# Keep-Passion/ImageStitch

Hardware: AMD Instinct MI355X
Metric: image-pairs/sec (2048x2048 grayscale, SURF+BF) (higher is better)
Workload: dtype f32

## Files before the change

imagestitch_amd/csrc/surf_kernels.hip:

```cpp
#include "common.h"
#include "detmath.h"
#include <math.h>
#include <float.h>
#include <string.h>
#include <stdlib.h>
#include <algorithm>
#include <vector>

#define GAS __attribute__((address_space(1)))
typedef GAS const uint8_t *g_cu8;
typedef GAS const int32_t *g_ci32;
typedef GAS float *g_f32;
typedef GAS const float *g_cf32;
typedef GAS int32_t *g_i32;
__device__ __forceinline__ int cv_round_f(float v) { return (int)rintf(v); }
__device__ __forceinline__ uint8_t round_u8_pos(float v) { return (uint8_t)__float_as_uint(v + 12582912.f); }
__device__ __forceinline__ int cv_round_d(double v) { return (int)rint(v); }
__device__ __forceinline__ int cv_floor_d(double v) { return (int)floor(v); }
__device__ __forceinline__ int cv_ceil_d(double v) { return (int)ceil(v); }

__device__ __forceinline__ int wave_incl_scan(int v)
{
    const int lane = threadIdx.x & 63;
#pragma unroll
// ... 863 lines not shown
#pragma unroll
                for (int off = 32; off >= 1; off >>= 1) {
                    const float om = __shfl_xor(bm, off, 64); const int oi = __shfl_xor(bi, off, 64);
                    if (om > bm || (om == bm && oi < bi)) { bm = om; bi = oi; }
                }
                if (lane == 0) {
                    float bestx = 0, besty = 0;
                    if (bm > 0.f) { bestx = sx_s[q][bi]; besty = sy_s[q][bi]; }
                    R.kps[k].angle = fast_atan2_deg(-besty, bestx);
                }
            }
        }
    }
}

#ifdef VFSMS_DESC_TIMING
__device__ unsigned long long g_desc_cycles[8];
#define DT_MARK(ph) do { if (threadIdx.x == 0) { unsigned long long _n = clock64(); atomicAdd(&g_desc_cycles[ph], _n - _t0); _t0 = _n; } } while (0)
#define DT_START unsigned long long _t0 = clock64()
extern "C" int vfsms_debug_desc_cycles(unsigned long long *out) { return hipMemcpyFromSymbol(out, HIP_SYMBOL(g_desc_cycles), sizeof(unsigned long long) * 8) == hipSuccess ? 0 : -3; }
__device__ unsigned long long g_desc_trips[4];
#define DT_TRIP(n) do {} while (0)
__device__ unsigned long long g_desc_unit_cycles[4];
#define DT_UNIT_BEGIN unsigned long long _u0 = clock64()
#define DT_UNIT_END(n) do { _uacc[n] += clock64() - _u0; _ucnt[n]++; } while (0)
extern "C" int vfsms_debug_desc_unit_cycles(unsigned long long *out) { return hipMemcpyFromSymbol(out, HIP_SYMBOL(g_desc_unit_cycles), sizeof(unsigned long long) * 4) == hipSuccess ? 0 : -3; }
extern "C" int vfsms_debug_desc_trips(unsigned long long *out) { return hipMemcpyFromSymbol(out, HIP_SYMBOL(g_desc_trips), sizeof(unsigned long long) * 4) == hipSuccess ? 0 : -3; }
#else
#define DT_MARK(ph) do {} while (0)
#define DT_START do {} while (0)
#define DT_TRIP(n) do {} while (0)
#define DT_UNIT_BEGIN do {} while (0)
#define DT_UNIT_END(n) do {} while (0)
#endif
#ifndef VFSMS_EXP
#define VFSMS_EXP 0
#endif
#ifndef DESC_WBUF
#define DESC_WBUF 15360
#endif
__device__ __forceinline__ void origin_chain(float *row, float s, const float d, const int n)
{
    int i = 0;
    for (; i + 4 <= n; i += 4) {
        const float a = s, b = a + d, c = b + d, e = c + d;
        s = e + d;
        row[i] = a; row[i + 1] = b; row[i + 2] = c; row[i + 3] = e;
    }
    for (; i < n; i++, s += d) row[i] = s;
}

struct WinGeom {
    int win; float sin_dir, cos_dir;
    int h, w, stride; g_cu8 img;
    g_cu8 pair;
    int upright, usx, usy;
};

__device__ __forceinline__ int win_sample_xy(const WinGeom &G, double px, double py)
{
    const int ncols1 = G.w - 1, nrows1 = G.h - 1;
    const int ix = (int)px, iy = (int)py;
    if (px >= 0.0 && py >= 0.0 && ix < ncols1 && iy < nrows1) {
        const float a = (float)__builtin_amdgcn_fract(px), b = (float)__builtin_amdgcn_fract(py);
        g_cu8 p = G.img + (size_t)iy * G.stride + ix;
        const float v = p[0] * (1.f - a) * (1.f - b) + p[1] * a * (1.f - b) + p[G.stride] * (1.f - a) * b + p[G.stride + 1] * a * b;
        return (int)(uint8_t)cv_round_f(v);
    }
    const int x = min(max(cv_round_d(px), 0), ncols1);
    const int y = min(max(cv_round_d(py), 0), nrows1);
    return (int)G.img[(size_t)y * G.stride + x];
}
__device__ __forceinline__ int win_sample_upright(const WinGeom &G, int i, int j)
{
    const int x = min(max(G.usx + i, 0), G.w - 1);
    const int y = min(max(G.usy - j, 0), G.h - 1);
    return (int)G.img[(size_t)y * G.stride + x];
}

typedef float float2v __attribute__((ext_vector_type(2)));
__device__ __forceinline__ float bilinear_pk(uint32_t top, float a, float b)
{
    const float na = 1.f - a, nb = 1.f - b;
    const float2v w = {na, a};
    const float2v r0 = {(float)(top & 0xff), (float)((top >> 16) & 0xff)};
    const float2v r1 = {(float)((top >> 8) & 0xff), (float)(top >> 24)};
    float2v p = r0 * w, q = r1 * w;
    const float2v nb2 = {nb, nb}, b2 = {b, b};
    p = p * nb2; q = q * b2;
    return ((p.x + p.y) + q.x) + q.y;
}
#ifndef STAGE_ILP
#define STAGE_ILP 4
#endif
#define UNIT_W (8 * STAGE_ILP)
#ifndef BORDER_ILP
#define BORDER_ILP 2
#endif
#ifndef STAGE_FRAC_FIRST
#define STAGE_FRAC_FIRST 1
#endif
template <int N>
__device__ __forceinline__ void stage_round(g_cu8 ubase, const uint32_t pw, const double c, const double sn, const double sxc, const double syc,
                                            const int jlane, uint8_t *wrow)
{
    uint32_t top[N];
    const double jd = (double)jlane;
    const double px0 = __builtin_fma(jd, c, sxc), py0 = __builtin_fma(jd, -sn, syc);
#if STAGE_FRAC_FIRST
    float fa[N], fb[N];
#pragma unroll
    for (int u = 0; u < N; u++) {
        const double px = u ? px0 + (double)(8 * u) * c : px0, py = u ? py0 - (double)(8 * u) * sn : py0;
        const uint32_t off = ((uint32_t)__umul24((uint32_t)(int)py, pw) + (uint32_t)(int)px) << 1;
        fa[u] = (float)__builtin_amdgcn_fract(px); fb[u] = (float)__builtin_amdgcn_fract(py);
        top[u] = *(GAS const uint32_t *)(ubase + off);
    }
#pragma unroll
    for (int u = 0; u < N; u++) wrow[8 * u] = round_u8_pos(bilinear_pk(top[u], fa[u], fb[u]));
#else
    double px[N], py[N];
    px[0] = px0; py[0] = py0;
#pragma unroll
    for (int u = 1; u < N; u++) { px[u] = px[0] + (double)(8 * u) * c; py[u] = py[0] - (double)(8 * u) * sn; }
#pragma unroll
    for (int u = 0; u < N; u++) {
        const uint32_t off = ((uint32_t)__umul24((uint32_t)(int)py[u], pw) + (uint32_t)(int)px[u]) << 1;
        top[u] = *(GAS const uint32_t *)(ubase + off);
    }
#pragma unroll
    for (int u = 0; u < N; u++) {
        const float a = (float)__builtin_amdgcn_fract(px[u]), b = (float)__builtin_amdgcn_fract(py[u]);
        wrow[8 * u] = round_u8_pos(bilinear_pk(top[u], a, b));
    }
#endif
}

template <int NW>
__device__ __forceinline__ void stage_rows(const WinGeom &G, const float *sx_row, const float *sy_row,
                                           int r0, int nrows, uint8_t *dst, uint8_t *strip_in)
{
    const int win = __builtin_amdgcn_readfirstlane(G.win);
    r0 = __builtin_amdgcn_readfirstlane(r0); nrows = __builtin_amdgcn_readfirstlane(nrows);
    const int lane = threadIdx.x & 63, wv = NW == 1 ? 0 : __builtin_amdgcn_readfirstlane((int)(threadIdx.x >> 6));
    const int li = lane >> 3, lj = lane & 7;
    const int strips = (nrows + 7) >> 3;
    const double c = (double)G.cos_dir, sn = (double)G.sin_dir;
    const int ncols1 = __builtin_amdgcn_readfirstlane(G.w) - 1, nrows1 = __builtin_amdgcn_readfirstlane(G.h) - 1;
    const uint64_t bp = (uint64_t)G.pair;
    g_cu8 ubase = (g_cu8)(((uint64_t)(uint32_t)__builtin_amdgcn_readfirstlane((uint32_t)(bp >> 32)) << 32) |
                          (uint64_t)(uint32_t)__builtin_amdgcn_readfirstlane((uint32_t)bp));
    const uint32_t pw = (uint32_t)(ncols1 + 1);
    const int gfull = win >> 3, tailc = win & 7;
    int nb = NW == 1 ? 1 : (gfull + 7) >> 3;
#if VFSMS_EXP & 16
    nb = (gfull + 3) >> 2;
#endif
    const int gbase = gfull / nb, grem = gfull - gbase * nb;
    const int total = strips * nb;
    if (!G.upright) {
        const int tid = NW == 1 ? lane : (int)threadIdx.x;
        if (tid < strips) {
            const int ia = min(r0 + tid * 8, VFSMS_MAX_WIN - 1), ib = min(min(r0 + tid * 8 + 7, r0 + nrows - 1), VFSMS_MAX_WIN - 1);
            const double xa = (double)sx_row[ia], xb = (double)sx_row[ib], ya = (double)sy_row[ia], yb = (double)sy_row[ib];
            const double jb = (double)(win - 1);
            const double jxb = jb * c, jyb = -(jb * sn);
            const double xmin = fmin(xa, xb) + fmin(0.0, jxb), xmax = fmax(xa, xb) + fmax(0.0, jxb);
            const double ymin = fmin(ya, yb) + fmin(0.0, jyb), ymax = fmax(ya, yb) + fmax(0.0, jyb);
            strip_in[tid] = xmin >= 0.0 && ymin >= 0.0 && xmax < (double)(ncols1 - 2) && ymax < (double)nrows1;
        }
        if (NW == 1) { __builtin_amdgcn_fence(__ATOMIC_ACQ_REL, "wavefront"); __builtin_amdgcn_wave_barrier(); }
        else __syncthreads();
    }
    int ty = 0, cbi = wv;
    while (cbi >= nb) { cbi -= nb; ty++; }
#ifdef VFSMS_DESC_TIMING
    unsigned long long _s0 = clock64(), _uacc[2] = {0, 0}, _ucnt[2] = {0, 0};
#endif
    const int last_row = r0 + nrows - 1;
    const int liw = li * win;
    const int last_off = (nrows - 1) * win;
    float nsx = 0.f, nsy = 0.f; int nflag = 0;
    if (wv < total) {
        const int ic0 = min(r0 + ty * 8 + li, last_row);
        nsx = sx_row[ic0]; nsy = sy_row[ic0]; nflag = strip_in[ty];
    }
    for (int unit = wv; unit < total; unit += NW) {
        DT_UNIT_BEGIN;
        const int g0 = cbi * gbase + min(cbi, grem), gn = gbase + (cbi < grem ? 1 : 0);
        const bool last_run = cbi == nb - 1;
        const int cb0 = g0 * 8;
        const int cb1 = last_run ? win : cb0 + gn * 8;
        const double sxc = (double)nsx, syc = (double)nsy;
        const int flag_cur = nflag;
        const int ty_cur = ty;
        uint8_t *drc = dst + min(ty * 8 * win + liw, last_off);
        cbi += NW;
        while (cbi >= nb) { cbi -= nb; ty++; }
        if (unit + NW < total) {
            const int icn = min(r0 + ty * 8 + li, last_row);
            nsx = sx_row[icn]; nsy = sy_row[icn]; nflag = strip_in[ty];
        }
        if (G.upright) {
            for (int j = cb0 + lj; j < cb1; j += 8) drc[j] = (uint8_t)win_sample_upright(G, min(r0 + ty_cur * 8 + li, last_row), j);
            continue;
        }
        bool unit_in = __builtin_amdgcn_readfirstlane(flag_cur) != 0;
        if (!unit_in) {
            const int ia = min(r0 + ty_cur * 8, VFSMS_MAX_WIN - 1), ib = min(min(r0 + ty_cur * 8 + 7, last_row), VFSMS_MAX_WIN - 1);
            const double xa = (double)sx_row[ia], xb = (double)sx_row[ib], ya = (double)sy_row[ia], yb = (double)sy_row[ib];
            const double ja = (double)cb0, jb = (double)(cb1 - 1);
            const double jxa = ja * c, jxb = jb * c, jya = -(ja * sn), jyb = -(jb * sn);
            const double xmin = fmin(xa, xb) + fmin(jxa, jxb), xmax = fmax(xa, xb) + fmax(jxa, jxb);
            const double ymin = fmin(ya, yb) + fmin(jya, jyb), ymax = fmax(ya, yb) + fmax(jya, jyb);
            unit_in = xmin >= 0.0 && ymin >= 0.0 && xmax < (double)(ncols1 - 2) && ymax < (double)nrows1;
        }
        if (unit_in) {
            DT_TRIP(0);
            uint8_t *wrow = drc + cb0 + lj;
            int jl = cb0 + lj, left = gn;
            while (left >= 4) { stage_round<4>(ubase, pw, c, sn, sxc, syc, jl, wrow); jl += 32; wrow += 32; left -= 4; }
            if (left == 3) stage_round<3>(ubase, pw, c, sn, sxc, syc, jl, wrow);
            else if (left == 2) stage_round<2>(ubase, pw, c, sn, sxc, syc, jl, wrow);
            else if (left == 1) stage_round<1>(ubase, pw, c, sn, sxc, syc, jl, wrow);
            if (last_run && tailc) {
                const int jc = min(gfull * 8 + lj, win - 1);
                stage_round<1>(ubase, pw, c, sn, sxc, syc, jc, drc + jc);
            }
            DT_UNIT_END(0);
            continue;
        }
        DT_TRIP(2);
        for (int jb = cb0; jb < cb1; jb += 8 * BORDER_ILP) {
            double px[BORDER_ILP], py[BORDER_ILP];
            int jc[BORDER_ILP];
            uint32_t top[BORDER_ILP];
            bool inside[BORDER_ILP];
#pragma unroll
            for (int u = 0; u < BORDER_ILP; u++) {
                jc[u] = min(jb + u * 8 + lj, cb1 - 1);
                px[u] = sxc + (double)jc[u] * c;
                py[u] = syc - (double)jc[u] * sn;
                const int ix = (int)px[u], iy = (int)py[u];
                inside[u] = px[u] >= 0.0 && py[u] >= 0.0 && ix < ncols1 && iy < nrows1;
                const int rx = min(max(cv_round_d(px[u]), 0), ncols1), ry = min(max(cv_round_d(py[u]), 0), nrows1);
                const int cx = inside[u] ? ix : rx, cy = inside[u] ? iy : ry;
                top[u] = *(GAS const uint32_t *)(ubase + (((uint32_t)__umul24((uint32_t)cy, pw) + (uint32_t)cx) << 1));
            }
#pragma unroll
            for (int u = 0; u < BORDER_ILP; u++) {
                const float a = (float)__builtin_amdgcn_fract(px[u]), b = (float)__builtin_amdgcn_fract(py[u]);
                const float v = (float)(top[u] & 0xff) * (1.f - a) * (1.f - b) + (float)((top[u] >> 16) & 0xff) * a * (1.f - b) +
                                (float)((top[u] >> 8) & 0xff) * (1.f - a) * b + (float)(top[u] >> 24) * a * b;
                drc[jc[u]] = inside[u] ? (uint8_t)cv_round_f(v) : (uint8_t)(top[u] & 0xff);
            }
        }
        DT_UNIT_END(1);
    }
#ifdef VFSMS_DESC_TIMING
    if ((threadIdx.x & 63) == 0) {
        atomicAdd(&g_desc_unit_cycles[2], clock64() - _s0);
        atomicAdd(&g_desc_unit_cycles[0], _uacc[0]); atomicAdd(&g_desc_unit_cycles[1], _uacc[1]);
        atomicAdd(&g_desc_trips[0], _ucnt[0]); atomicAdd(&g_desc_trips[2], _ucnt[1]);
    }
#endif
}

__device__ __forceinline__ uint8_t sat_u8(float v)
{
    int iv = cv_round_f(v);
    return (uint8_t)(iv < 0 ? 0 : iv > 255 ? 255 : iv);
}

struct AreaRec { int j0, n; float a0, af, al; int mode, r1, r2; };
#define AREA_RECS 22

__device__ __forceinline__ float area_row_tab(const uint8_t *S, const AreaRec &c, const int nmin, const int nmax)
{
    const uint8_t *p = S + c.j0;
    float buf = (float)p[0] * c.a0;
    int t = 1;
    for (; t < nmin - 1; t++) buf += (float)p[t] * c.af;
    for (; t < nmax; t++) buf += (float)p[t] * (t < c.n - 1 ? c.af : (t == c.n - 1 ? c.al : 0.f));
    return buf;
}
#define AREA_TAIL 4
__device__ __forceinline__ void area_tail_weights(const AreaRec &c, const int nmin, float (&w)[AREA_TAIL])
{
    const int t0 = max(nmin - 1, 1);
#pragma unroll
    for (int i = 0; i < AREA_TAIL; i++) w[i] = t0 + i < c.n - 1 ? c.af : (t0 + i == c.n - 1 ? c.al : 0.f);
}
__device__ __forceinline__ float area_row_tab_w(const uint8_t *S, const AreaRec &c, const int nmin, const int nmax, const float (&w)[AREA_TAIL])
{
    const uint8_t *p = S + c.j0;
    float buf = (float)p[0] * c.a0;
    int t = 1;
    for (; t < nmin - 1; t++) buf += (float)p[t] * c.af;
#pragma unroll
    for (int i = 0; i < AREA_TAIL; i++)
        if (t + i < nmax) buf += (float)p[t + i] * w[i];
    return buf;
}
__device__ __forceinline__ uint8_t area_col_tab(const float *rb, const AreaRec &c, const int mode, const float inv_area)
{
    float sum = c.a0 * rb[0];
    for (int t = 1; t < c.n; t++) sum += (t < c.n - 1 ? c.af : c.al) * rb[t * 21];
    if (mode == 2) return (uint8_t)(((int)sum + 2) >> 2);
    if (mode == 1) return sat_u8(sum * inv_area);
    return sat_u8(sum);
}

__device__ void describe_one(const RoiDev &R, const SurfTables *T, const AreaRec *area_tab, const DescRec &rec, int extended, int upright, const int band)
{
    DT_START;
    const int k = rec.k;
    __shared__ float sx_row[VFSMS_MAX_WIN], sy_row[VFSMS_MAX_WIN];
    __shared__ uint8_t PATCH[21][21 + 3];
    __shared__ AreaRec REC[AREA_RECS];
    __shared__ uint8_t WINBUF[DESC_WBUF];
    __shared__ float rowsum[40 * 21];
    __shared__ uint8_t STRIP_IN[VFSMS_MAX_WIN / 8 + 8];
    WinGeom G;
    G.win = max(21, min(rec.win, VFSMS_MAX_WIN));
    G.h = R.h; G.w = R.w; G.stride = R.stride; G.img = (g_cu8)R.img; G.pair = (g_cu8)R.pair;
    G.upright = upright; G.usx = 0; G.usy = 0; G.sin_dir = rec.sin_dir; G.cos_dir = rec.cos_dir;
    const int win = G.win;
    const int dsz = 21;
    if (threadIdx.x < AREA_RECS * 8) ((int *)REC)[threadIdx.x] = ((const int *)(area_tab + (size_t)win * AREA_RECS))[threadIdx.x];
    __syncthreads();
    const int nmin = __builtin_amdgcn_readfirstlane(REC[21].j0), nmax = __builtin_amdgcn_readfirstlane(REC[21].n);
    const int mode = __builtin_amdgcn_readfirstlane(REC[21].mode);
    const float inv_area = REC[21].a0;
    if (!upright) {
        if (threadIdx.x == 0 || threadIdx.x == 64) {
            const float sin_dir = rec.sin_dir, cos_dir = rec.cos_dir;
            const float win_offset = -(float)(win - 1) / 2;
            const int need = band >= 0 ? min(win, REC[band].j0 + REC[band].n) : win;
            if (threadIdx.x == 0) origin_chain(sx_row, rec.x + win_offset * cos_dir + win_offset * sin_dir, sin_dir, need);
            else origin_chain(sy_row, rec.y - win_offset * sin_dir + win_offset * cos_dir, cos_dir, need);
        }
    } else {
        const float win_offset = -(float)(win - 1) / 2;
        G.usx = cv_round_f(rec.x + win_offset);
        G.usy = cv_round_f(rec.y - win_offset);
    }
    __syncthreads();
    DT_MARK(0);

    const bool tail_ok = nmax - max(nmin - 1, 1) <= AREA_TAIL;
    auto reduce_rows = [&](const int st_lo, int dyA, const int dy_stop) {
        while (dyA < dy_stop) {
            const int lo = REC[dyA].j0;
            int dyB = dyA + 1;
            while (dyB < dy_stop && REC[dyB].j0 + REC[dyB].n - lo <= 40) dyB++;
            const int nr = REC[dyB - 1].j0 + REC[dyB - 1].n - lo;
            for (int e = threadIdx.x; e < nr * 21; e += 256) {
                const int r = (int)(((uint32_t)e * 3121u) >> 16), dx = e - 21 * r;
                if (tail_ok) {
                    const AreaRec cx = REC[dx];
                    float w[AREA_TAIL];
                    area_tail_weights(cx, nmin, w);
                    rowsum[e] = area_row_tab_w(WINBUF + (lo - st_lo + r) * win, cx, nmin, nmax, w);
                } else
                    rowsum[e] = area_row_tab(WINBUF + (lo - st_lo + r) * win, REC[dx], nmin, nmax);
            }
            __syncthreads();
            for (int o = threadIdx.x; o < (dyB - dyA) * 21; o += 256) {
                const int dyl = (int)(((uint32_t)o * 3121u) >> 16), dx = o - 21 * dyl;
                const AreaRec ry = REC[dyA + dyl];
                PATCH[dyA + dyl][dx] = area_col_tab(rowsum + (ry.j0 - lo) * 21 + dx, ry, mode, inv_area);
            }
            __syncthreads();
            dyA = dyB;
        }
    };
    if (win * win <= DESC_WBUF) {
        stage_rows<4>(G, sx_row, sy_row, 0, win, WINBUF, STRIP_IN);
        __syncthreads();
        DT_MARK(1);
        reduce_rows(0, 0, dsz);
        DT_MARK(2);
    } else {
        const int dy_end = band >= 0 ? band + 1 : dsz;
        const int crows = max(DESC_WBUF / win, 1);
        for (int dy = band >= 0 ? band : 0; dy < dy_end;) {
            const int rlo = REC[dy].j0, nrows = REC[dy].n;
            if (nrows <= crows) {
                int d_stop = dy + 1;
                while (d_stop < dy_end && REC[d_stop].j0 + REC[d_stop].n - rlo <= crows) d_stop++;
                const int end = REC[d_stop - 1].j0 + REC[d_stop - 1].n - 1;
                stage_rows<4>(G, sx_row, sy_row, rlo, end - rlo + 1, WINBUF, STRIP_IN);
                __syncthreads();
                DT_MARK(3);
                reduce_rows(rlo, dy, d_stop);
                DT_MARK(4);
                dy = d_stop;
            } else {
                for (int c0 = 0; c0 < nrows; c0 += crows) {
                    const int cn = min(crows, nrows - c0);
                    stage_rows<4>(G, sx_row, sy_row, rlo + c0, cn, WINBUF, STRIP_IN);
                    __syncthreads();
                    DT_MARK(3);
                    for (int e = threadIdx.x; e < cn * 21; e += 256) {
                        const int r = (int)(((uint32_t)e * 3121u) >> 16), dx = e - 21 * r;
                        rowsum[c0 * 21 + e] = area_row_tab(WINBUF + r * win, REC[dx], nmin, nmax);
                    }
                    __syncthreads();
                }
                if (threadIdx.x < dsz) PATCH[dy][threadIdx.x] = area_col_tab(rowsum + threadIdx.x, REC[dy], mode, inv_area);
                __syncthreads();
                DT_MARK(4);
                dy++;
            }
        }
    }
    __syncthreads();
    if (band >= 0) {
        if (threadIdx.x < 21) R.patch[(size_t)k * VFSMS_PATCH_ROW + band * 21 + threadIdx.x] = PATCH[band][threadIdx.x];
    } else {
        for (int o = threadIdx.x; o < 441; o += 256) R.patch[(size_t)k * VFSMS_PATCH_ROW + o] = PATCH[o / 21][o % 21];
    }
    DT_MARK(5);
}

#define DESC_NCLS 4

__device__ __forceinline__ int desc_class(float size)
{
    const float s = size * 1.2f / 9.0f;
    const int win = min((int)((20 + 1) * s), VFSMS_MAX_WIN);
    return win > 256 ? 0 : win > 128 ? 1 : win > 64 ? 2 : 3;
}

__global__ __launch_bounds__(1024) void k_desc_order(const RoiDev *rois)
{
    const RoiDev &R = rois[blockIdx.x];
    const int n = min(R.counters[0], R.cap);
    __shared__ int cnt[DESC_NCLS], base[DESC_NCLS], cur[DESC_NCLS];
    if (threadIdx.x < DESC_NCLS) { cnt[threadIdx.x] = 0; cur[threadIdx.x] = 0; }
    __syncthreads();
    const int lane = threadIdx.x & 63;
    for (int k0 = 0; k0 < n; k0 += 1024) {
        const int k = k0 + threadIdx.x;
        const float size = k < n ? R.kps[k].size : -1.f;
        const int cls = size > 0 ? desc_class(size) : -1;
#pragma unroll
        for (int c = 0; c < DESC_NCLS; c++) {
            const unsigned long long m = __ballot(cls == c);
            if (m && lane == __ffsll((long long)m) - 1) atomicAdd(&cnt[c], __popcll(m));
        }
    }
    __syncthreads();
    if (threadIdx.x == 0) {
        int acc = 0;
        for (int c = 0; c < DESC_NCLS; c++) { base[c] = acc; acc += cnt[c]; R.counters[12 + c] = cnt[c]; }
    }
    __syncthreads();
    for (int k0 = 0; k0 < n; k0 += 1024) {
        const int k = k0 + threadIdx.x;
        const float size = k < n ? R.kps[k].size : -1.f;
        const int cls = size > 0 ? desc_class(size) : -1;
#pragma unroll
        for (int c = 0; c < DESC_NCLS; c++) {
            const unsigned long long m = __ballot(cls == c);
            if (!m) continue;
            const int leader = __ffsll((long long)m) - 1;
            int start = 0;
            if (lane == leader) start = atomicAdd(&cur[c], __popcll(m));
            start = __shfl(start, leader, 64);
            if (cls == c) R.order[base[c] + start + __popcll(m & ((1ull << lane) - 1))] = k;
        }
    }
}

#define DESC_HEADS DESC_PLAN_HEADS
#define DESC_HEAD_STRIDE 64

__global__ __launch_bounds__(256) void k_desc_plan(const RoiDev *rois, int nrois, DescPlan *plan, int big_grid)
{
    __shared__ int c[VFSMS_MAX_ROIS][4];
    for (int e = threadIdx.x; e < nrois * 4; e += 256) c[e >> 2][e & 3] = rois[e >> 2].counters[12 + (e & 3)];
    __syncthreads();
    if (threadIdx.x == 0) {
        int acc = 0, total = 0;
        for (int q = 0; q < DESC_HEADS; q++) {
            plan->big_start[q] = acc;
            for (int r = q; r < nrois; r += DESC_HEADS) { plan->seg_base[r][0] = acc; acc += c[r][0]; }
            plan->big_n0[q] = acc - plan->big_start[q];
            for (int r = q; r < nrois; r += DESC_HEADS) {
                plan->seg_base[r][1] = acc; acc += c[r][1];
                plan->seg_base[r][2] = acc; acc += c[r][2];
            }
            plan->big_tickets[q] = acc - plan->big_start[q];
        }
        total = acc;
        const int split = total < big_grid * 48 ? 21 : 1;
        plan->split = split;
        for (int q = 0; q < DESC_HEADS; q++) plan->big_tickets[q] += (split - 1) * plan->big_n0[q];
        acc = 0;
        for (int q = 0; q < DESC_HEADS; q++) {
            plan->small_start[q] = acc;
            for (int r = q; r < nrois; r += DESC_HEADS) { plan->seg_base[r][3] = acc; acc += c[r][3]; }
            plan->small_tickets[q] = acc - plan->small_start[q];
        }
    }
}

__global__ __launch_bounds__(256) void k_desc_recs(const RoiDev *rois, const DescPlan *plan, DescRec *big, DescRec *small, int upright)
{
    const int roi = blockIdx.y;
    const RoiDev &R = rois[roi];
    const int p = blockIdx.x * 256 + threadIdx.x;
    const int c0 = R.counters[12], c1 = R.counters[13], c2 = R.counters[14], c3 = R.counters[15];
    if (p >= c0 + c1 + c2 + c3) return;
    const int cls = p < c0 ? 0 : p < c0 + c1 ? 1 : p < c0 + c1 + c2 ? 2 : 3;
    const int idx = p - (cls > 0 ? c0 : 0) - (cls > 1 ? c1 : 0) - (cls > 2 ? c2 : 0);
    const int k = R.order[p];
    const vfsms_keypoint kp = R.kps[k];
    DescRec rec;
    rec.roi = roi; rec.k = k; rec.pad = 0; rec.x = kp.x; rec.y = kp.y;
    rec.win = (int)((20 + 1) * (kp.size * 1.2f / 9.0f));
    rec.sin_dir = 0.f; rec.cos_dir = 0.f;
    if (!upright) {
        const float dir = kp.angle * (float)(3.1415926535897932384626433832795 / 180);
        double sd, cd;
        det_sincos((double)dir, &sd, &cd);
        rec.sin_dir = -(float)sd;
        rec.cos_dir = (float)cd;
    }
    (cls < 3 ? big : small)[plan->seg_base[roi][cls] + idx] = rec;
}

__global__ __launch_bounds__(ORI_KP * 128, 8) void k_orientation(const RoiDev *rois, const SurfTables *T, int upright)
{
    const RoiDev &R = rois[blockIdx.y];
    const int n = min(R.counters[0], R.cap);
    const int k0 = blockIdx.x * ORI_KP;
    if (k0 >= n) return;
    orientation_block(R, T, k0, n, upright);
}

#define DESC_SMALL_WIN 64
struct SmallLds { uint8_t win[DESC_SMALL_WIN * DESC_SMALL_WIN + 64]; float sx[DESC_SMALL_WIN + 8], sy[DESC_SMALL_WIN + 8]; AreaRec rec[AREA_RECS]; int rec_win; uint8_t strip_in[DESC_SMALL_WIN / 8 + 8]; };

__device__ __forceinline__ void wave_sync_lds()
{
    __builtin_amdgcn_fence(__ATOMIC_ACQ_REL, "wavefront");
    __builtin_amdgcn_wave_barrier();
}

__device__ void describe_small(const RoiDev &R, const AreaRec *area_tab, const DescRec &rec, int upright, SmallLds &L)
{
    const int lane = threadIdx.x & 63;
    const int k = rec.k;
    WinGeom G;
    G.win = min(rec.win, DESC_SMALL_WIN);
    G.h = R.h; G.w = R.w; G.stride = R.stride; G.img = (g_cu8)R.img; G.pair = (g_cu8)R.pair;
    G.upright = upright; G.usx = 0; G.usy = 0; G.sin_dir = rec.sin_dir; G.cos_dir = rec.cos_dir;
    const int win = G.win;
    const int dsz = 21;
    if (L.rec_win != win) {
        wave_sync_lds();
        const int *src = (const int *)(area_tab + (size_t)max(win, dsz) * AREA_RECS);
        for (int e = lane; e < AREA_RECS * 8; e += 64) ((int *)L.rec)[e] = src[e];
        if (lane == 0) L.rec_win = win;
    }
    if (!upright) {
        const float sin_dir = rec.sin_dir, cos_dir = rec.cos_dir;
        if (lane < 2) {
            const float win_offset = -(float)(win - 1) / 2;
            const float sx0 = rec.x + win_offset * cos_dir + win_offset * sin_dir, sy0 = rec.y - win_offset * sin_dir + win_offset * cos_dir;
            origin_chain(lane == 0 ? L.sx : L.sy, lane == 0 ? sx0 : sy0, lane == 0 ? sin_dir : cos_dir, win);
        }
    } else {
        const float win_offset = -(float)(win - 1) / 2;
        G.usx = cv_round_f(rec.x + win_offset);
        G.usy = cv_round_f(rec.y - win_offset);
    }
    wave_sync_lds();
    stage_rows<1>(G, L.sx, L.sy, 0, win, L.win, L.strip_in);
    wave_sync_lds();
    const int nmin = __builtin_amdgcn_readfirstlane(L.rec[21].j0), nmax = __builtin_amdgcn_readfirstlane(L.rec[21].n);
    const int mode = __builtin_amdgcn_readfirstlane(L.rec[21].mode);
    const float inv_area = L.rec[21].a0;
    const bool tail_ok = nmax - max(nmin - 1, 1) <= AREA_TAIL;
    uint8_t *prow = R.patch + (size_t)k * VFSMS_PATCH_ROW;
    for (int o = lane; o < dsz * dsz; o += 64) {
        const int dy = (int)(((uint32_t)o * 3121u) >> 16), dx = o - dsz * dy;
        const AreaRec ry = L.rec[dy], rx = L.rec[dx];
        const uint8_t *S = L.win + ry.j0 * win;
        float sum;
        if (tail_ok) {
            float w[AREA_TAIL];
            area_tail_weights(rx, nmin, w);
            sum = ry.a0 * area_row_tab_w(S, rx, nmin, nmax, w);
            for (int ty = 1; ty < nmax; ty++) {
                const float beta = ty < ry.n - 1 ? ry.af : (ty == ry.n - 1 ? ry.al : 0.f);
                sum += beta * area_row_tab_w(S + ty * win, rx, nmin, nmax, w);
            }
        } else {
            sum = ry.a0 * area_row_tab(S, rx, nmin, nmax);
            for (int ty = 1; ty < nmax; ty++) {
                const float beta = ty < ry.n - 1 ? ry.af : (ty == ry.n - 1 ? ry.al : 0.f);
                sum += beta * area_row_tab(S + ty * win, rx, nmin, nmax);
            }
        }
        uint8_t outv;
        if (mode == 2) outv = (uint8_t)(((int)sum + 2) >> 2);
        else if (mode == 1) outv = sat_u8(sum * inv_area);
        else outv = sat_u8(sum);
        prow[o] = outv;
    }
    wave_sync_lds();
}

#ifndef DESC_SMALL_WGS
#define DESC_SMALL_WGS 7
#endif
__device__ __forceinline__ DescRec load_rec_uniform(const DescRec *p)
{
    const int *q = (const int *)p;
    DescRec r;
    r.roi = __builtin_amdgcn_readfirstlane(q[0]); r.k = __builtin_amdgcn_readfirstlane(q[1]);
    r.win = __builtin_amdgcn_readfirstlane(q[2]); r.pad = 0;
    r.sin_dir = __int_as_float(__builtin_amdgcn_readfirstlane(q[4])); r.cos_dir = __int_as_float(__builtin_amdgcn_readfirstlane(q[5]));
    r.x = __int_as_float(__builtin_amdgcn_readfirstlane(q[6])); r.y = __int_as_float(__builtin_amdgcn_readfirstlane(q[7]));
    return r;
}
__global__ __launch_bounds__(256, DESC_SMALL_WGS) void k_describe_small(const RoiDev *rois, const DescPlan *plan, const DescRec *recs, int *counter,
                                                                 const AreaRec *area_tab, int upright)
{
    __shared__ SmallLds L[4];
    if (threadIdx.x < 4) L[threadIdx.x].rec_win = -1;
    __syncthreads();
    const int lane = threadIdx.x & 63, wave = __builtin_amdgcn_readfirstlane((int)(threadIdx.x >> 6));
    int head = 0;
    for (;;) {
        int slot = -1;
        if (lane == 0)
            while (head < DESC_HEADS) {
                const int q = (blockIdx.x + head) & (DESC_HEADS - 1);
                const int n = plan->small_tickets[q];
                const int t = n > 0 ? atomicAdd(counter + q * DESC_HEAD_STRIDE, 1) : 0;
                if (t < n) { slot = plan->small_start[q] + t; break; }
                head++;
            }
        slot = __builtin_amdgcn_readfirstlane(slot);
        head = __builtin_amdgcn_readfirstlane(head);
        if (slot < 0) break;
        const DescRec rec = load_rec_uniform(recs + slot);
        describe_small(rois[rec.roi], area_tab, rec, upright, L[wave]);
    }
}

__global__ __launch_bounds__(256) void k_pair_rows(const RoiDev *rois)
{
    const RoiDev &R = rois[blockIdx.z];
    const int y = blockIdx.y, x = (blockIdx.x * 256 + threadIdx.x) * 4;
    if (y >= R.h || x >= R.w) return;
    g_cu8 r0 = (g_cu8)R.img + (size_t)y * R.stride + x, r1 = (g_cu8)R.img + (size_t)min(y + 1, R.h - 1) * R.stride + x;
    GAS uint16_t *dst = (GAS uint16_t *)R.pair + (size_t)y * R.w + x;
    if (x + 4 <= R.w) {
        const uint32_t a = *(GAS const u32u *)r0, b = *(GAS const u32u *)r1;
#pragma unroll
        for (int k = 0; k < 4; k++) dst[k] = (uint16_t)(((a >> (8 * k)) & 0xff) | (((b >> (8 * k)) & 0xff) << 8));
    } else {
        for (int k = 0; x + k < R.w; k++) dst[k] = (uint16_t)(r0[k] | (r1[k] << 8));
    }
}

#ifndef DESC_WGS
#define DESC_WGS 6
#endif
__global__ __launch_bounds__(256, DESC_WGS) void k_describe(const RoiDev *rois, const DescPlan *plan, const DescRec *recs, int *counter, const SurfTables *T,
                                                  const AreaRec *area_tab, int extended, int upright)
{
    __shared__ int s_slot, s_band;
    int head = 0;
#ifdef VFSMS_DESC_TIMING
    unsigned long long tq = clock64();
#endif
    for (;;) {
        __syncthreads();
        if (threadIdx.x == 0) {
            int slot = -1, band = -1;
            const int split = plan->split;
            while (head < DESC_HEADS) {
                const int q = (blockIdx.x + head) & (DESC_HEADS - 1);
                const int n = plan->big_tickets[q];
                const int t = n > 0 ? atomicAdd(counter + q * DESC_HEAD_STRIDE, 1) : 0;
                if (t < n) {
                    const int n0 = plan->big_n0[q];
                    if (t < n0 * split) { slot = plan->big_start[q] + t / split; band = split > 1 ? t % split : -1; }
                    else slot = plan->big_start[q] + n0 + (t - n0 * split);
                    break;
                }
                head++;
            }
            s_slot = slot; s_band = band;
        }
        __syncthreads();
        const int slot = __builtin_amdgcn_readfirstlane(s_slot), band = __builtin_amdgcn_readfirstlane(s_band);
        if (slot < 0) break;
#ifdef VFSMS_DESC_TIMING
        if (threadIdx.x == 0) atomicAdd(&g_desc_cycles[6], clock64() - tq);
#endif
        const DescRec rec = load_rec_uniform(recs + slot);
        describe_one(rois[rec.roi], T, area_tab, rec, extended, upright, band);
#ifdef VFSMS_DESC_TIMING
        tq = clock64();
#endif
    }
}

__global__ __launch_bounds__(1024) void k_keep_scan(const RoiDev *rois)
{
// ... 318 lines not shown
```

Measured before the change: 2304.

## Stream large descriptor windows in uniform row chunks with running column accumulators

Replaces the per-output-row staging of oversized descriptor windows with a single pass over the needed row range, in chunks sized to leave room for a 441-float accumulator carved from the window buffer. Row sums are computed in passes of 36 rows and folded into per-output-pixel partial column sums, so rows shared by neighbouring output rows are staged only once and chunk counts drop. It also uses the precomputed tail-weight row reduction when allowed. The cost is extra accumulator traffic, more synchronisation inside each chunk, and a smaller usable staging buffer.

```diff
diff --git a/imagestitch_amd/csrc/surf_kernels.hip b/imagestitch_amd/csrc/surf_kernels.hip
--- a/imagestitch_amd/csrc/surf_kernels.hip
+++ b/imagestitch_amd/csrc/surf_kernels.hip
@@ -1189,14 +1189,20 @@
         if (t + i < nmax) buf += (float)p[t + i] * w[i];
     return buf;
 }
-__device__ __forceinline__ uint8_t area_col_tab(const float *rb, const AreaRec &c, const int mode, const float inv_area)
-{
-    float sum = c.a0 * rb[0];
-    for (int t = 1; t < c.n; t++) sum += (t < c.n - 1 ? c.af : c.al) * rb[t * 21];
+__device__ __forceinline__ uint8_t area_out(const float sum, const int mode, const float inv_area)
+{
     if (mode == 2) return (uint8_t)(((int)sum + 2) >> 2);
     if (mode == 1) return sat_u8(sum * inv_area);
     return sat_u8(sum);
 }
+__device__ __forceinline__ uint8_t area_col_tab(const float *rb, const AreaRec &c, const int mode, const float inv_area)
+{
+    float sum = c.a0 * rb[0];
+    for (int t = 1; t < c.n; t++) sum += (t < c.n - 1 ? c.af : c.al) * rb[t * 21];
+    return area_out(sum, mode, inv_area);
+}
+#define DESC_ACC_OFF (DESC_WBUF - 441 * 4)
+#define DESC_PASS 36
 
 __device__ void describe_one(const RoiDev &R, const SurfTables *T, const AreaRec *area_tab, const DescRec &rec, int extended, int upright, const int band)
 {
@@ -1269,37 +1275,47 @@
         reduce_rows(0, 0, dsz);
         DT_MARK(2);
     } else {
-        const int dy_end = band >= 0 ? band + 1 : dsz;
-        const int crows = max(DESC_WBUF / win, 1);
-        for (int dy = band >= 0 ? band : 0; dy < dy_end;) {
-            const int rlo = REC[dy].j0, nrows = REC[dy].n;
-            if (nrows <= crows) {
-                int d_stop = dy + 1;
-                while (d_stop < dy_end && REC[d_stop].j0 + REC[d_stop].n - rlo <= crows) d_stop++;
-                const int end = REC[d_stop - 1].j0 + REC[d_stop - 1].n - 1;
-                stage_rows<4>(G, sx_row, sy_row, rlo, end - rlo + 1, WINBUF, STRIP_IN);
+        float *acc = (float *)(WINBUF + DESC_ACC_OFF);
+        const int dyA = band >= 0 ? band : 0, dyB = band >= 0 ? band + 1 : dsz;
+        const int rlo = REC[dyA].j0, rhi = REC[dyB - 1].j0 + REC[dyB - 1].n;
+        const int crows = (DESC_ACC_OFF / win) & ~7;
+        for (int c0 = rlo; c0 < rhi; c0 += crows) {
+            const int cn = min(crows, rhi - c0);
+            stage_rows<4>(G, sx_row, sy_row, c0, cn, WINBUF, STRIP_IN);
+            __syncthreads();
+            DT_MARK(3);
+            for (int p0 = 0; p0 < cn; p0 += DESC_PASS) {
+                const int pn = min(DESC_PASS, cn - p0);
+                for (int e = threadIdx.x; e < pn * 21; e += 256) {
+                    const int r = (int)(((uint32_t)e * 3121u) >> 16), dx = e - 21 * r;
+                    if (tail_ok) {
+                        const AreaRec cx = REC[dx];
+                        float w[AREA_TAIL];
+                        area_tail_weights(cx, nmin, w);
+                        rowsum[e] = area_row_tab_w(WINBUF + (p0 + r) * win, cx, nmin, nmax, w);
+                    } else
+                        rowsum[e] = area_row_tab(WINBUF + (p0 + r) * win, REC[dx], nmin, nmax);
+                }
                 __syncthreads();
-                DT_MARK(3);
-                reduce_rows(rlo, dy, d_stop);
-                DT_MARK(4);
-                dy = d_stop;
-            } else {
-                for (int c0 = 0; c0 < nrows; c0 += crows) {
-                    const int cn = min(crows, nrows - c0);
-                    stage_rows<4>(G, sx_row, sy_row, rlo + c0, cn, WINBUF, STRIP_IN);
-                    __syncthreads();
-                    DT_MARK(3);
-                    for (int e = threadIdx.x; e < cn * 21; e += 256) {
-                        const int r = (int)(((uint32_t)e * 3121u) >> 16), dx = e - 21 * r;
-                        rowsum[c0 * 21 + e] = area_row_tab(WINBUF + r * win, REC[dx], nmin, nmax);
+                const int s0 = c0 + p0, s1 = s0 + pn;
+                for (int o = threadIdx.x; o < 441; o += 256) {
+                    const int dy = (int)(((uint32_t)o * 3121u) >> 16), dx = o - 21 * dy;
+                    const AreaRec ry = REC[dy];
+                    const int a = max(ry.j0, s0), b = min(ry.j0 + ry.n, s1);
+                    if (dy < dyA || dy >= dyB || a >= b) continue;
+                    float sum = a == ry.j0 ? 0.f : acc[o];
+                    for (int s = a; s < b; s++) {
+                        const int t = s - ry.j0;
+                        const float rb = rowsum[(s - s0) * 21 + dx];
+                        if (t == 0) sum = ry.a0 * rb;
+                        else sum += (t < ry.n - 1 ? ry.af : ry.al) * rb;
                     }
-                    __syncthreads();
+                    if (b == ry.j0 + ry.n) PATCH[dy][dx] = area_out(sum, mode, inv_area);
+                    else acc[o] = sum;
                 }
-                if (threadIdx.x < dsz) PATCH[dy][threadIdx.x] = area_col_tab(rowsum + threadIdx.x, REC[dy], mode, inv_area);
-                __syncthreads();
-                DT_MARK(4);
-                dy++;
-            }
+                if (p0 + DESC_PASS < cn) __syncthreads();
+            }
+            DT_MARK(4);
         }
     }
     __syncthreads();
```

Result: faster. 2353 (median of 6 runs) (+2.1%).
